# zhaorz/FlowOnTheGo

Measured on AMD Instinct MI355X. Metric: frame-pairs/sec @1080p DIS op-pt 2 (4 batches of 64 in flight), higher is better.
Workload: dtype f32; 1 GPU; BASELINE configs[2]: batch 64 synthetic 1920x1080 gray f32 pairs per GPU resident in HBM, DIS op-pt 2 + variational refinement (SOR order: lexicographic = the reference's order), output = finest-scale flow 120x68x2; global_batch=64, pairs_in_flight=256, batches_in_flight_per_gpu=4, parallelism=frame-pair sharding x1, no collective

## Files before the change

### flowonthego_amd/csrc/fotg_capi.hip

```cpp
#include <math.h>
#include <stdio.h>
#include <stdlib.h>
#include <string.h>
#include <atomic>
#include <map>
#include <mutex>
#include <new>
#include <type_traits>
#include "host_call.h"
#include "pipe_tickets.h"
#include "pipe_queues.h"
#include "pyramid.hip.h"
#include "lk.hip.h"
#include "lk_fast.hip.h"
#include "densify.hip.h"
#include "varref.hip.h"
#include "varref_tiles.hip.h"
#include "varref_levelpipe.hip.h"
#include "varref_depth.hip.h"
#include "upsample.hip.h"

using namespace fotg;

static thread_local int g_last_hip = 0;
// ... 1 lines not shown
#define HIPCHK(x)                                   \
  do {                                              \
    hipError_t e_ = (x);                            \
    if (e_ != hipSuccess) { g_last_hip = (int)e_; return FOTG_ERR_HIP; } \
  } while (0)
#define LAUNCHCHK() HIPCHK(hipGetLastError())

#define ON_DEVICE(dev)                                                              \
  DevGuard dev_guard_(dev);                                                         \
  if (!dev_guard_.ok) { g_last_hip = (int)hipGetLastError(); return FOTG_ERR_HIP; }

struct GridState {
  const float *I0, *I0x, *I0y, *I1;
  long stride;
  const float *flow_prev;
  float *trace_host;
  int camlr;
};
struct Grid {
  float *p_iter[FOTG_MAXLEV];
  float *pweight[FOTG_MAXLEV];
  GridState gs[FOTG_MAXLEV];
};
struct PyrBufs {
  float *im[FOTG_MAXLEV], *dx[FOTG_MAXLEV], *dy[FOTG_MAXLEV];
};

struct FotgTune {
  int vr_path;
  int vr_stream;
  int vr_levelpipe;
  int lp_max_pairs;
  int vr_first_data;
  int pyr_split;
  int lk_shw;
  int lk_lpp;
  int lk_banded;
  int lk_fast_r;
  int lk_lpp_min_waves;
  int test_taps;
};
static const char *env_str(const char *name) { return getenv(name); }
static int env_int(const char *name, int dflt) { const char *e = env_str(name); return e ? atoi(e) : dflt; }

#ifdef FOTG_DEBUG
static std::map<void *, void *> g_dbg_base;
static std::mutex g_dbg_mu;
static hipError_t fotg_dbg_free(void *p)
{
  void *base = p;
  { std::lock_guard<std::mutex> g(g_dbg_mu); auto it = g_dbg_base.find(p); if (it != g_dbg_base.end()) { base = it->second; g_dbg_base.erase(it); } }
  return (hipFree)(base);
}
#define hipFree(p) fotg_dbg_free((void *)(p))
#endif
struct fotg_ctx {
#ifdef FOTG_DEBUG
  struct Guard { const char *name; char *begin, *end; size_t size; } guards[256];
  int nguards;
#endif
  fotg_params p;
  FotgTune tune;
  int w_org, h_org, Wp, Hp, padw, padh, device, max_batch, noc, ps;
  int nch;
  int base_lv;
  LevelGeom geom[FOTG_MAXLEV];
  PyrBufs pyr[2];
  long lev_stride[FOTG_MAXLEV];
  float *flow[FOTG_MAXLEV];
  Grid fw;
  Grid bw;
  float *flow_bw[FOTG_MAXLEV];
  float *tap_t[FOTG_MAXLEV], *tap_tx[FOTG_MAXLEV], *tap_ty[FOTG_MAXLEV], *tap_hes[FOTG_MAXLEV];
  int *tap_cnt[FOTG_MAXLEV];
  float *trace_dev[FOTG_MAXLEV];
  bool taps;
  float *vr;
  long vr_pair_stride;
  float4 *vrC[FOTG_MAXLEV];
  float2 *vrD[FOTG_MAXLEV];
  VrArgs vra[FOTG_MAXLEV];
  int verbosity;
  hipEvent_t tev[4 * FOTG_MAXLEV + 4];
  float tt[FOTG_MAXLEV][5];
  float tt_pyr, tt_total;
  float2 *vrX[FOTG_MAXLEV];
  long x_pair_stride[FOTG_MAXLEV];
  int x_rt[FOTG_MAXLEV];
  int *tileSync;
  long sync_total;
  int tile_nbs;
  int lp_ntr;
  int *stall_host, *stall_dev;
  long stalls;
  unsigned long long *stamps;
};
// ... 94 lines not shown
    (void)hipFree(c->trace_dev[l]);
    (void)hipFree(c->vrC[l]); (void)hipFree(c->vrD[l]); (void)hipFree(c->vrX[l]);
  }
  if (c->stall_host) (void)hipHostFree(c->stall_host);
  (void)hipFree(c->vr); (void)hipFree(c->tileSync); (void)hipFree(c->stamps);
  for (auto &e : c->tev) if (e) (void)hipEventDestroy(e);
  delete c;
}

int fotg_create(const fotg_params *p, int w_org, int h_org, int device, int max_batch, fotg_ctx **out)
{
  if (!p || !out || w_org <= 0 || h_org <= 0 || max_batch <= 0) return FOTG_ERR_ARG;
  if (p->noc != 1 && p->noc != 3) return FOTG_ERR_ARG;
  if (p->ps != 4 && p->ps != 8 && p->ps != 12 && p->ps != 16) return FOTG_ERR_UNSUPPORTED;
  if (p->sc_l < 0 || p->sc_f < p->sc_l || p->sc_f >= FOTG_MAXLEV) return FOTG_ERR_ARG;
  if (p->max_iter < 0 || p->tv_solverit < 0 || p->tv_innerit < 0) return FOTG_ERR_ARG;
  if (p->costfct < 0 || p->costfct > 2 || (p->costfct == 2 && !(p->normoutlier > 0))) return FOTG_ERR_ARG;
  if (p->depth && p->usetvref && p->sor_mode != FOTG_SOR_LEXICOGRAPHIC) return FOTG_ERR_UNSUPPORTED;
  if (p->sor_mode < FOTG_SOR_LEXICOGRAPHIC || p->sor_mode > FOTG_SOR_POINT) return FOTG_ERR_ARG;
  if (p->u8_color < 0 || p->u8_color > 2 || (p->u8_color && p->noc != 1)) return FOTG_ERR_ARG;
  if (p->bidir != 0 && p->bidir != 1) return FOTG_ERR_ARG;
  if (p->bidir && p->depth) return FOTG_ERR_UNSUPPORTED;
  ON_DEVICE(device);
  fotg_ctx *c = new (std::nothrow) fotg_ctx();
  if (!c) return FOTG_ERR_ARG;
  memset((void *)c, 0, sizeof(*c));
  c->p = *p; c->w_org = w_org; c->h_org = h_org; c->device = device; c->max_batch = max_batch;
  c->noc = p->noc; c->ps = p->ps; c->nch = p->depth ? 1 : 2;
  c->tune.vr_path = env_int("FOTG_VR_PATH", 0);
  c->tune.vr_stream = env_int("FOTG_VR_STREAM", 1);
  c->tune.vr_levelpipe = env_int("FOTG_VR_LEVELPIPE", 1);
  c->tune.lp_max_pairs = env_int("FOTG_VR_LEVELPIPE_MAX_PAIRS", 1 << 20);
  c->tune.vr_first_data = env_int("FOTG_VR_FIRST_DATA", 1);
  c->tune.pyr_split = env_int("FOTG_PYR_SPLIT", 1);
  c->tune.test_taps = env_int("FOTG_TEST_TAPS", 0);
  c->tune.lk_shw = env_int("FOTG_LK_SHW", -1);
  c->tune.lk_lpp = env_int("FOTG_LK_LPP", 0);
  c->tune.lk_banded = env_int("FOTG_LK_BANDED", 1);
  c->tune.lk_lpp_min_waves = env_int("FOTG_LK_LPP_MIN_WAVES", 2048);
  c->tune.lk_fast_r = env_int("FOTG_LK_FAST_R", 2);
  if (hipHostMalloc((void **)&c->stall_host, 64, hipHostMallocMapped) != hipSuccess ||
      hipHostGetDevicePointer((void **)&c->stall_dev, c->stall_host, 0) != hipSuccess) { g_last_hip = (int)hipGetLastError(); fotg_destroy(c); return FOTG_ERR_HIP; }
  memset(c->stall_host, 0, 64);
  fotg_padded_size(w_org, h_org, p->sc_f, &c->Wp, &c->Hp, &c->padw, &c->padh);
  c->base_lv = p->sc_l < 4 ? p->sc_l : 4;
  const size_t B = (size_t)max_batch;
  for (int l = c->base_lv; l <= p->sc_f; ++l) {
    LevelGeom &g = c->geom[l];
    fill_geom(*p, c->Wp, c->Hp, l, g);
    if (g.w < 1 || g.h < 1) { fotg_destroy(c); return FOTG_ERR_ARG; }
    c->lev_stride[l] = (long)g.tw * g.th * c->noc;
    const size_t bytes = B * c->lev_stride[l] * sizeof(float);
#ifdef FOTG_DEBUG
#define FOTG_GUARD_BYTES 65536
#define ALLOC(ptr, nbytes) do { const bool gd_ = getenv("FOTG_DEBUG_GUARD") != nullptr; const size_t nb_ = ((nbytes) + 255) & ~(size_t)255; char *base_ = nullptr; \
    if (hipMalloc((void **)&base_, nb_ + (gd_ ? 2 * FOTG_GUARD_BYTES : 0)) != hipSuccess) { g_last_hip = (int)hipGetLastError(); fotg_destroy(c); return FOTG_ERR_HIP; } \
    *(void **)&(ptr) = gd_ ? base_ + FOTG_GUARD_BYTES : base_; \
    if (getenv("FOTG_DEBUG_POISON")) (void)hipMemset((ptr), getenv("FOTG_DEBUG_POISON")[0] == '2' ? 0x4B : 0xFF, nb_); \
    if (gd_ && c->nguards < 256) { (void)hipMemset(base_, 0xA5, FOTG_GUARD_BYTES); (void)hipMemset(base_ + FOTG_GUARD_BYTES + nb_, 0xA5, FOTG_GUARD_BYTES); \
      { std::lock_guard<std::mutex> g_(g_dbg_mu); g_dbg_base[(void *)(ptr)] = base_; } \
      c->guards[c->nguards].name = #ptr; c->guards[c->nguards].begin = base_; c->guards[c->nguards].end = base_ + FOTG_GUARD_BYTES + nb_; c->guards[c->nguards++].size = nb_; } } while (0)
#else
#define ALLOC(ptr, nbytes) do { if (hipMalloc((void **)&(ptr), (nbytes)) != hipSuccess) { g_last_hip = (int)hipGetLastError(); fotg_destroy(c); return FOTG_ERR_HIP; } } while (0)
#endif
    const size_t bytes1 = (B + 1) * c->lev_stride[l] * sizeof(float);
    ALLOC(c->pyr[0].im[l], bytes1);
// ... 533 lines not shown
  const int npx = a.w * a.h;
  if (mode != FOTG_SOR_POINT && c->tune.vr_path == 0 && inner >= 1 && sync_bands(a, sweeps) == 1 && fused_lds_bytes(a, false) <= 156 * 1024 &&
      (npx <= 3000 || mode == FOTG_SOR_REDBLACK)) {
    p.nsweeps = nosor ? 0 : sweeps;
    p.fused = fused_lds_bytes(a, true) > FOTG_LDS_MAX ? FUSED_CGLOBAL
            : c->noc == 1 && npx > 1024 && npx <= 2048 ? FUSED_RES1024
            : c->noc == 1 && npx <= 1024 ? FUSED_RES
            : FUSED_CL;
    p.lds = fused_lds_bytes(a, p.fused != FUSED_CGLOBAL);
    return p;
  }
  p.merged_first = c->tune.vr_first_data && inner > 0;
  const bool tiled = c->vrX[l] && c->tileSync;
  const int ntr = (a.h + FOTG_LP_TH - 1) / FOTG_LP_TH;
  const long lp_words = lp_tile_words(n, c->tile_nbs) + lp_data_words(n, ntr);
  p.levelpipe = tiled && c->tune.vr_levelpipe && n <= c->tune.lp_max_pairs && c->tune.vr_path == 0 && c->tune.vr_first_data &&
                inner >= 1 && inner <= FOTG_LP_KMAX && sweeps >= 2 && sweeps <= 4 && ntr <= c->lp_ntr && lp_words <= c->sync_total;
  p.zsync_n = !tiled ? 0 : p.levelpipe ? (int)lp_words : (int)tile_sync_words(n, c->tile_nbs);
  if (p.levelpipe) {
    const int nb = (a.h + FOTG_TILE_ROWS - 1) / FOTG_TILE_ROWS;
    p.lp_nwg = (unsigned)n * (unsigned)(inner * nb * sweeps + (inner - 1) * ntr * FOTG_LP_DW);
    p.excl = (p.lp_nwg <= 256 && !((c->tune.vr_levelpipe >> 4) & 8)) ? 72 * 1024 : 0;
  }
  return p;
}

template <typename... A>
static int opt_in_lds(void (*fn)(A...), int lds)
{
  HIPCHK(lds_opt_in(fn, lds));
  return FOTG_OK;
}

enum LaunchCount { CNT_SOR_STREAM, CNT_SOR_PIPE, CNT_FUSED_CGLOBAL, CNT_SOR_TILES, CNT_SOR_TALL, CNT_LEVEL_PIPE, CNT_N };
static const char *const g_count_name[CNT_N] = {"sor_stream", "sor_pipe", "fused_cglobal", "sor_tiles", "sor_tall", "level_pipe"};
static std::atomic<long> g_count[CNT_N];

#ifndef FOTG_TILE_P
#define FOTG_TILE_P 8
#endif
static TileArgs tile_args(const fotg_ctx *c, int l, int n)
{
  const VrArgs &a = c->vra[l];
  return {c->vrX[l], c->x_pair_stride[l], (long)(a.S + 1 + FOTG_TILE_DUMP) * c->x_rt[l], c->x_rt[l], (a.h + FOTG_TILE_ROWS - 1) / FOTG_TILE_ROWS, n,
          c->tileSync, c->tile_nbs, c->tileSync + c->sync_total, c->stall_dev};
}

template <int K, int P, bool POINT = false>
static void launch_sor_wave(const VrArgs &a, int n, int sweeps, float omega, hipStream_t s)
{
  constexpr int U = POINT ? (K <= 4 ? 4 : 1) : (K <= 2) ? (P >= 8 ? 64 : 8 * P) : (K <= 4 ? 4 * P : P);
  vr_sor_kernel<K, P, U, POINT><<<n, 64, 0, s>>>(a, sweeps, omega);
}

template <bool FM>
static int run_sor(fotg_ctx *c, int l, int n, const SorPlan &q, bool zeroed, hipStream_t s)
{
  const VrArgs &a = c->vra[l];
  const int sweeps = c->p.tv_solverit;
  const float omega = c->p.tv_sor;
  int st = FOTG_OK;
  switch (q.kind) {
    case SOR_NONE: return FOTG_OK;
    case SOR_STREAM70:
      if ((st = opt_in_lds(vr_sor_stream_kernel<72, 70, FOTG_SYNC_M, kVrU, FM>, q.lds))) return st;
      vr_sor_stream_kernel<72, 70, FOTG_SYNC_M, kVrU, FM><<<n, 1024, q.lds, s>>>(with_bands(a, q.nsweeps, q.nbands), omega);
      ++g_count[CNT_SOR_STREAM];
      break;
    case SOR_STREAM98:
// ... 64 lines not shown

template <int NOC, bool FM>
static int varref_impl(fotg_ctx *c, int l, int n, const float *I0, const float *I1, long img_stride, float *flow, hipStream_t s)
{
  const LevelGeom &g = c->geom[l];
  const VrArgs &a = c->vra[l];
  const long fs = (long)g.w * g.h * 2;
  dim3 grid((g.w * g.h + 255) / 256, n), block(256);
  const float quarter_alpha = 0.25f * c->p.tv_alpha;
  const float half_gamma_over3 = c->p.tv_gamma * 0.5f / 3.0f;
  const float half_delta_over3 = c->p.tv_delta * 0.5f / 3.0f;
  const int inner = c->p.tv_innerit * (l + 1);
  const VrPlan p = plan_level(c, l, n);
  int st = FOTG_OK;
  if (p.fused != FUSED_NONE) {
    VrArgs b = with_bands(a, p.nsweeps, 1);
    b.taps = c->taps ? 1 : 0;
    b.redblack = c->p.sor_mode == FOTG_SOR_REDBLACK;
    const auto fused = [&](auto launch) {
      return launch(b, p.lds, n, s, inner, quarter_alpha, half_delta_over3, half_gamma_over3, c->p.tv_sor, flow, fs, I0, I1, img_stride, g.tw, c->ps);
    };
    switch (p.fused) {
      case FUSED_RES1024: if constexpr (NOC == 1) st = fused(launch_fused<1, true, true, 1024, FM>); break;
      case FUSED_RES: if constexpr (NOC == 1) st = fused(launch_fused<1, true, true, 512, FM>); break;
      case FUSED_CL: st = fused(launch_fused<NOC, true, false, 512, FM>); break;
      default: st = fused(launch_fused<NOC, false, false, 512, FM>); ++g_count[CNT_FUSED_CGLOBAL]; break;
    }
    if (st) return st;
    LAUNCHCHK();
    return FOTG_OK;
  }
  VrArgs az = a;
  if (p.zsync_n) { az.zsync = c->tileSync; az.zsync_n = p.zsync_n; }
  {
    dim3 gs_(((g.w + 31) / 32) * ((g.h + 7) / 8), n);
    if ((n & 7) != 0 && gs_.x >= 256 && c->tune.lk_banded) { az.nwg = (int)gs_.x; gs_.x = (gs_.x + 7) & ~7u; }
    vr_setup_kernel<NOC, 2, FM><<<gs_, 256, 0, s>>>(az, I0, I1, img_stride, g.tw, c->ps, flow, fs, 1, p.merged_first ? 1 : 0, quarter_alpha, half_delta_over3, half_gamma_over3);
    LAUNCHCHK();
  }
  if (p.levelpipe) {
    LevelPipeArgs q;
    q.K = inner; q.ntr = (g.h + FOTG_LP_TH - 1) / FOTG_LP_TH; q.tiles_x = (g.w + FOTG_TW - 1) / FOTG_TW;
    q.dprog = c->tileSync + lp_tile_words(n, c->tile_nbs);
    q.quarter_alpha = quarter_alpha; q.half_delta_over3 = half_delta_over3; q.half_gamma_over3 = half_gamma_over3;
    q.dbg = c->tune.vr_levelpipe >> 4;
    q.stamps = nullptr;
    if (q.dbg & 4) {
      if (!c->stamps && hipMalloc((void **)&c->stamps, 8 * 8 * 8192) != hipSuccess) return FOTG_ERR_HIP;
      (void)hipMemsetAsync(c->stamps, 0, 8 * 8 * 8192, s);
      q.stamps = (long long *)c->stamps;
    }
    if (p.excl && (st = opt_in_lds(vr_level_pipe_kernel<NOC, FOTG_TILE_P, FM>, p.excl))) return st;
    vr_level_pipe_kernel<NOC, FOTG_TILE_P, FM><<<p.lp_nwg, 256, p.excl, s>>>(a, tile_args(c, l, n), q, c->p.tv_solverit, c->p.tv_sor);
    LAUNCHCHK();
    ++g_count[CNT_LEVEL_PIPE];
    vr_finish_kernel<<<grid, block, 0, s>>>(a, flow, fs);
    LAUNCHCHK();
    return FOTG_OK;
  }
  for (int it = 0; it < inner; ++it) {
    if (!(it == 0 && p.merged_first)) {
      vr_data_kernel<NOC, FM><<<dim3(((g.w + FOTG_TW - 1) / FOTG_TW) * ((g.h + FOTG_TH - 1) / FOTG_TH), n), 256, 0, s>>>(az, quarter_alpha, half_delta_over3, half_gamma_over3);
      LAUNCHCHK();
    }
    if ((st = run_sor<FM>(c, l, n, p.sor, p.zsync_n != 0, s))) return st;
  }
  vr_finish_kernel<<<grid, block, 0, s>>>(a, flow, fs);
  LAUNCHCHK();
  return FOTG_OK;
}

// ... 17 lines not shown
  else if (split && p.lds_mode) p.kind = DE_SPLIT;
  else p.kind = c->p.tv_solverit == 3 ? DE_SW3 : DE_SW1;
  return p;
}

template <int SW, bool SPLIT = false>
static int launch_de_sor(const VrArgs &a, int n, const DePlan &p, float omega, int camlr, hipStream_t s)
{
  const int nt = SPLIT ? 3 * p.threads : p.threads;
  int st = FOTG_OK;
  switch (p.lds_mode) {
    case 2: if (!(st = opt_in_lds(vr_de_sor_kernel<SW, 2, SPLIT>, p.lds))) vr_de_sor_kernel<SW, 2, SPLIT><<<n, nt, p.lds, s>>>(a, omega, camlr); break;
    case 1: if (!(st = opt_in_lds(vr_de_sor_kernel<SW, 1, SPLIT>, p.lds))) vr_de_sor_kernel<SW, 1, SPLIT><<<n, nt, p.lds, s>>>(a, omega, camlr); break;
    default: if constexpr (!SPLIT) vr_de_sor_kernel<SW, 0><<<n, nt, 0, s>>>(a, omega, camlr); break;
  }
  return st;
}

template <int NOC>
static int varref_depth_impl(fotg_ctx *c, int l, int n, const float *I0, const float *I1, long img_stride, float *flow, hipStream_t s, int camlr)
{
  const LevelGeom &g = c->geom[l];
  const VrArgs &a = c->vra[l];
  const long fs = (long)g.w * g.h;
  dim3 grid((g.w * g.h + 255) / 256, n), block(256);
  const float quarter_alpha = 0.25f * c->p.tv_alpha;
  const float half_gamma_over3 = c->p.tv_gamma * 0.5f / 3.0f;
  const float half_delta_over3 = c->p.tv_delta * 0.5f / 3.0f;
  const int inner = c->p.tv_innerit * (l + 1);
  const int sweeps = c->p.tv_solverit;
  const float omega = c->p.tv_sor;
  const DePlan p = plan_depth(c, l);
  int st = FOTG_OK;
  vr_setup_kernel<NOC, 1><<<dim3(((g.w + 31) / 32) * ((g.h + 7) / 8), n), 256, 0, s>>>(a, I0, I1, img_stride, g.tw, c->ps, flow, fs);
  LAUNCHCHK();
  if (p.kind == DE_INNER) {
    if ((st = opt_in_lds(vr_de_inner_kernel<NOC>, p.lds))) return st;
    vr_de_inner_kernel<NOC><<<n, 1024, p.lds, s>>>(a, inner, quarter_alpha, half_delta_over3, half_gamma_over3, omega, camlr, flow, fs, p.threads, c->taps ? 1 : 0);
    LAUNCHCHK();
    return FOTG_OK;
  }
  vr_de_init_kernel<<<grid, block, 0, s>>>(a);
  LAUNCHCHK();
  for (int it = 0; it < inner; ++it) {
    vr_de_smooth_kernel<<<grid, block, 0, s>>>(a, quarter_alpha);
    LAUNCHCHK();
    vr_de_data_kernel<NOC><<<grid, block, 0, s>>>(a, half_delta_over3, half_gamma_over3);
    LAUNCHCHK();
    switch (p.kind) {
      case DE_TALL:
        for (int k = 0; k < sweeps; ++k) vr_de_sor_tall_kernel<<<n, 1024, 0, s>>>(a, omega, camlr, k == sweeps - 1 ? 1 : 0);
        break;
      case DE_SPLIT: st = launch_de_sor<3, true>(a, n, p, omega, camlr, s); break;
      case DE_SW3: st = launch_de_sor<3>(a, n, p, omega, camlr, s); break;
      default: for (int k = 0; k < sweeps && !st; ++k) st = launch_de_sor<1>(a, n, p, omega, camlr, s); break;
    }
    if (st) return st;
    LAUNCHCHK();
  }
  vr_de_finish_kernel<<<grid, block, 0, s>>>(a, flow, fs);
  LAUNCHCHK();
  return FOTG_OK;
}

static int varref_dispatch(fotg_ctx *c, int l, int n, const float *I0, const float *I1, long pair_stride, float *flow, hipStream_t stream, int camlr)
{
  int st = check_level(c, l, n); if (st) return st;
  if (!I0 || !I1 || !flow || !c->vr) return FOTG_ERR_ARG;
// ... 703 lines not shown
```

### flowonthego_amd/csrc/varref.hip.h

```cpp
#pragma once
#include <type_traits>
#include "common.h"

namespace fotg {

enum VrPlane { P_WX = 0, P_WY, P_MASK, P_NSINGLE };
enum VrCPlane { C_AVG = 0, C_IZ, C_IX, C_IY, C_IXX, C_IXY, C_IYY, C_IXZ, C_IYZ, C_NCOLOR };

struct VrArgs {
  float *base;
  long pair_stride;
  long pl;
  int w, h, st, noc;
  float4 *C;
  float2 *D;
  long c_pair_stride;
  long d_pair_stride;
  int S, SC, RP, RPD, K, nlanes, nsweeps, nbands, band_rows, band_mode, taps;
  int *zsync;
  int zsync_n;
  int nwg;
  int redblack;
  int point;
  __host__ __device__ int pix(int i, int j) const { return j * st + i; }
// ... 72 lines not shown
__device__ __forceinline__ void prep_pixel(const VrArgs &a, int pair, int i, int j, const float *__restrict__ I0, const float *__restrict__ I1,
                                           long img_stride, int tw, int pad, const float *__restrict__ flow, long flow_stride)
{
  prep_store<NOC>(a, pair, i, j, prep_values<NOC>(a, pair, i, j, I0, I1, img_stride, tw, pad, flow, flow_stride));
}

template <int NOC>
__device__ __forceinline__ void deriv1_pixel(const VrArgs &a, int pair, int i, int j)
{
  const int o = j * a.st + i;
#pragma unroll
  for (int c = 0; c < NOC; ++c) {
    const float *avg = a.color(pair, C_AVG, c), *iz = a.color(pair, C_IZ, c);
    a.color(pair, C_IX, c)[o] = conv_h5(avg + (size_t)j * a.st, i, a.w);
    a.color(pair, C_IY, c)[o] = conv_v5(avg + i, j, a.h, a.st);
    a.color(pair, C_IXZ, c)[o] = conv_h5(iz + (size_t)j * a.st, i, a.w);
    a.color(pair, C_IYZ, c)[o] = conv_v5(iz + i, j, a.h, a.st);
  }
}

template <int NOC>
__device__ __forceinline__ void deriv2_pixel(const VrArgs &a, int pair, int i, int j)
{
  const int o = j * a.st + i;
#pragma unroll
  for (int c = 0; c < NOC; ++c) {
    const float *ix = a.color(pair, C_IX, c), *iy = a.color(pair, C_IY, c);
    a.color(pair, C_IXX, c)[o] = conv_h5(ix + (size_t)j * a.st, i, a.w);
    a.color(pair, C_IXY, c)[o] = conv_v5(ix + i, j, a.h, a.st);
    a.color(pair, C_IYY, c)[o] = conv_v5(iy + i, j, a.h, a.st);
  }
}

template <int NOC, int NCH, bool FM>
__device__ __forceinline__ void first_data_term(const VrArgs &a, int pair, int tx0, int ty0, const float *__restrict__ flow, long flow_stride,
                                                float quarter_alpha, float half_delta_over3, float half_gamma_over3);

template <int NOC, int NCH = 2, bool FM = false>
__global__ __launch_bounds__(256) void vr_setup_kernel(VrArgs a, const float *__restrict__ I0, const float *__restrict__ I1,
                                                       long img_stride, int tw, int pad,
                                                       const float *__restrict__ flow, long flow_stride, int zero_d = 0,
                                                       int first_data = 0, float quarter_alpha = 0.f, float half_delta_over3 = 0.f, float half_gamma_over3 = 0.f)
{
  constexpr int TW_ = 32, TH_ = 8, XW = TW_ + 8, XH = TH_ + 8, YW = TW_ + 4, YH = TH_ + 4;
  __shared__ float Xa[NOC][XH * XW], Xz[NOC][XH * XW], Yx[NOC][YH * YW], Yy[NOC][YH * YW];
  if (first_data && a.zsync_n > 0)
    for (long k = ((long)blockIdx.y * gridDim.x + blockIdx.x) * 256 + threadIdx.x; k < a.zsync_n; k += (long)gridDim.x * gridDim.y * 256) a.zsync[k] = 0;
  WgId wg = xcd_local_wg();
  int ntiles = (int)gridDim.x;
  if (a.nwg > 0) { wg.x = xcd_banded_x(a.nwg); ntiles = a.nwg; if (wg.x < 0) return; }
  const int pair = wg.y, w = a.w, h = a.h;
  const int tiles_x = (w + TW_ - 1) / TW_;
  if (zero_d == 1) {
    float2 *D = a.Dp(pair);
    for (long k = (long)wg.x * 256 + threadIdx.x; k < a.d_pair_stride; k += (long)ntiles * 256) D[k] = make_float2(0.f, 0.f);
  }
  const int tx0 = (wg.x % tiles_x) * TW_, ty0 = (wg.x / tiles_x) * TH_;
  for (int e = threadIdx.x; e < XW * XH; e += 256) {
    const int cx = tx0 - 4 + e % XW, cy = ty0 - 4 + e / XW;
    const int gx = clampi(cx, w), gy = clampi(cy, h);
    const PrepVal<NOC> v = prep_values<NOC, NCH>(a, pair, gx, gy, I0, I1, img_stride, tw, pad, flow, flow_stride);
#pragma unroll
    for (int c = 0; c < NOC; ++c) { Xa[c][e] = v.avg[c]; Xz[c][e] = v.iz[c]; }
    if (cx >= tx0 && cx < tx0 + TW_ && cy >= ty0 && cy < ty0 + TH_ && cx < w && cy < h) prep_store<NOC>(a, pair, cx, cy, v);
  }
  __syncthreads();
  for (int e = threadIdx.x; e < YW * YH; e += 256) {
    const int cx = tx0 - 2 + e % YW, cy = ty0 - 2 + e / YW;
    const int gx = clampi(cx, w), gy = clampi(cy, h);
    const bool own = cx >= tx0 && cx < tx0 + TW_ && cy >= ty0 && cy < ty0 + TH_ && cx < w && cy < h;
#pragma unroll
    for (int c = 0; c < NOC; ++c) {
      const float *arow = Xa[c] + (gy - ty0 + 4) * XW - tx0 + 4, *acol = Xa[c] + (4 - ty0) * XW + gx - tx0 + 4;
      const float *zrow = Xz[c] + (gy - ty0 + 4) * XW - tx0 + 4, *zcol = Xz[c] + (4 - ty0) * XW + gx - tx0 + 4;
      const float ix = conv_h5(arow, gx, w), iy = conv_v5(acol, gy, h, XW);
      const float ixz = conv_h5(zrow, gx, w), iyz = conv_v5(zcol, gy, h, XW);
      Yx[c][e] = ix; Yy[c][e] = iy;
      if (own) {
        const int o = a.pix(cx, cy);
        a.color(pair, C_IX, c)[o] = ix; a.color(pair, C_IY, c)[o] = iy; a.color(pair, C_IXZ, c)[o] = ixz; a.color(pair, C_IYZ, c)[o] = iyz;
      }
    }
  }
  __syncthreads();
  const int i = tx0 + (threadIdx.x % TW_), j = ty0 + (threadIdx.x / TW_);
  if (i < w && j < h) {
    const int o = a.pix(i, j);
#pragma unroll
    for (int c = 0; c < NOC; ++c) {
      const float *xrow = Yx[c] + (j - ty0 + 2) * YW - tx0 + 2, *xcol = Yx[c] + (2 - ty0) * YW + i - tx0 + 2, *ycol = Yy[c] + (2 - ty0) * YW + i - tx0 + 2;
      a.color(pair, C_IXX, c)[o] = conv_h5(xrow, i, w);
      a.color(pair, C_IXY, c)[o] = conv_v5(xcol, j, h, YW);
      a.color(pair, C_IYY, c)[o] = conv_v5(ycol, j, h, YW);
    }
  }
  if constexpr (NCH == 2) {
    if (first_data) {
      __syncthreads();
      first_data_term<NOC, NCH, FM>(a, pair, tx0, ty0, flow, flow_stride, quarter_alpha, half_delta_over3, half_gamma_over3);
    }
  }
}

template <int NOC>
struct PixIn {
  float Ix[NOC], Iy[NOC], Iz[NOC], Ixx[NOC], Ixy[NOC], Iyy[NOC], Ixz[NOC], Iyz[NOC];
  float m, wxc, wxl, wxr, wxt, wxb, wyc, wyl, wyr, wyt, wyb;
  __device__ __forceinline__ float dxl() const { return wxc - wxl; }
  __device__ __forceinline__ float dxr() const { return wxr - wxc; }
  __device__ __forceinline__ float dxt() const { return wxc - wxt; }
  __device__ __forceinline__ float dxb() const { return wxb - wxc; }
  __device__ __forceinline__ float dyl() const { return wyc - wyl; }
  __device__ __forceinline__ float dyr() const { return wyr - wyc; }
  __device__ __forceinline__ float dyt() const { return wyc - wyt; }
  __device__ __forceinline__ float dyb() const { return wyb - wyc; }
};
template <int NOC>
__device__ __forceinline__ PixIn<NOC> data_load(const VrArgs &a, int pair, int i, int j)
{
  const int st = a.st, w = a.w, h = a.h, o = j * st + i;
  const float *wx = a.single(pair, P_WX), *wy = a.single(pair, P_WY);
  PixIn<NOC> p;
#pragma unroll
  for (int c = 0; c < NOC; ++c) {
    p.Ix[c] = a.color(pair, C_IX, c)[o]; p.Iy[c] = a.color(pair, C_IY, c)[o]; p.Iz[c] = a.color(pair, C_IZ, c)[o];
    p.Ixx[c] = a.color(pair, C_IXX, c)[o]; p.Ixy[c] = a.color(pair, C_IXY, c)[o]; p.Iyy[c] = a.color(pair, C_IYY, c)[o];
    p.Ixz[c] = a.color(pair, C_IXZ, c)[o]; p.Iyz[c] = a.color(pair, C_IYZ, c)[o];
  }
  p.m = a.single(pair, P_MASK)[o];
  const int ol = i > 0 ? o - 1 : o, orr = i < w - 1 ? o + 1 : o, ot = j > 0 ? o - st : o, ob = j < h - 1 ? o + st : o;
  p.wxc = wx[o]; p.wxl = wx[ol]; p.wxr = wx[orr]; p.wxt = wx[ot]; p.wxb = wx[ob];
  p.wyc = wy[o]; p.wyl = wy[ol]; p.wyr = wy[orr]; p.wyt = wy[ot]; p.wyb = wy[ob];
  return p;
// ... 51 lines not shown
  const int x0 = (tile % tiles_x) * FOTG_TW, y0 = (tile / tiles_x) * FOTG_TH;
  const int lx = threadIdx.x % FOTG_TW, ly = threadIdx.x / FOTG_TW;
  const int i = x0 + lx, j = y0 + ly, o = j * st + i;
  const float *wx = a.single(pair, P_WX), *wy = a.single(pair, P_WY);
  const float2 *D = a.Dp(pair);
  const bool inimg = i < w && j < h;
  const int ic0 = inimg ? i : 0, jc0 = inimg ? j : 0;
  const PixIn<NOC> pin = data_load<NOC>(a, pair, ic0, jc0);
  const float2 duv = D[a.didx(ic0, jc0)];
  for (int k = threadIdx.x; k < UW * UH; k += 256) {
    const int jj = clampi(y0 - 2 + k / UW, h), ii = clampi(x0 - 2 + k % UW, w);
    const int q = jj * st + ii;
    const float2 d = D[a.didx(ii, jj)];
    uv[k] = make_float2(wx[q] + d.x, wy[q] + d.y);
  }
  __syncthreads();
  for (int k = threadIdx.x; k < SW * SH; k += 256) {
    const int sy = k / SW, sx = k % SW;
    const int c = (sy + 1) * UW + (sx + 1);
    sm[k] = smooth_w<FM>(uv[c - 1], uv[c], uv[c + 1], uv[c - UW], uv[c + UW], y0 - 1 + sy, h, quarter_alpha);
  }
  __syncthreads();
  if (i >= w || j >= h) return;
  const int sc = (ly + 1) * SW + (lx + 1);
  const float s_o = sm[sc];
  const float hr = (i < w - 1) ? s_o + sm[sc + 1] : 0.0f;
  const float hl = (i > 0) ? sm[sc - 1] + s_o : 0.0f;
  const float vb = (j < h - 1) ? s_o + sm[sc + SW] : 0.0f;
  const float vt = (j > 0) ? sm[sc - SW] + s_o : 0.0f;

  data_term_compute<NOC, FM>(a, pair, i, j, pin, hr, hl, vb, vt, duv.x, duv.y, half_delta_over3, half_gamma_over3);
}

template <int NOC, int NCH, bool FM>
__device__ __forceinline__ void first_data_term(const VrArgs &a, int pair, int x0, int y0, const float *__restrict__ flow, long flow_stride,
                                                float quarter_alpha, float half_delta_over3, float half_gamma_over3)
{
  constexpr int UW = FOTG_TW + 4, UH = FOTG_TH + 4, SW = FOTG_TW + 2, SH = FOTG_TH + 2;
  __shared__ float2 uv[UW * UH];
  __shared__ float sm[SW * SH];
  const int st = a.st, w = a.w, h = a.h;
  const int lx = threadIdx.x % FOTG_TW, ly = threadIdx.x / FOTG_TW;
  const int i = x0 + lx, j = y0 + ly;
  const float *fl = flow + (size_t)pair * flow_stride;
  auto W = [&](int ii, int jj) { const float *f = fl + NCH * (size_t)(jj * w + ii); return make_float2(f[0], f[NCH - 1]); };
  for (int k = threadIdx.x; k < UW * UH; k += 256) {
    const float2 wv = W(clampi(x0 - 2 + k % UW, w), clampi(y0 - 2 + k / UW, h));
    uv[k] = make_float2(wv.x + 0.f, wv.y + 0.f);
  }
  __syncthreads();
  for (int k = threadIdx.x; k < SW * SH; k += 256) {
    const int sy = k / SW, sx = k % SW;
    const int c = (sy + 1) * UW + (sx + 1);
    sm[k] = smooth_w<FM>(uv[c - 1], uv[c], uv[c + 1], uv[c - UW], uv[c + UW], y0 - 1 + sy, h, quarter_alpha);
  }
  __syncthreads();
  if (i >= w || j >= h) return;
  const int sc = (ly + 1) * SW + (lx + 1), o = j * st + i;
  const float s_o = sm[sc];
  const float hr = (i < w - 1) ? s_o + sm[sc + 1] : 0.0f;
  const float hl = (i > 0) ? sm[sc - 1] + s_o : 0.0f;
  const float vb = (j < h - 1) ? s_o + sm[sc + SW] : 0.0f;
  const float vt = (j > 0) ? sm[sc - SW] + s_o : 0.0f;
  PixIn<NOC> p;
#pragma unroll
  for (int c = 0; c < NOC; ++c) {
    p.Ix[c] = a.color(pair, C_IX, c)[o]; p.Iy[c] = a.color(pair, C_IY, c)[o]; p.Iz[c] = a.color(pair, C_IZ, c)[o];
    p.Ixx[c] = a.color(pair, C_IXX, c)[o]; p.Ixy[c] = a.color(pair, C_IXY, c)[o]; p.Iyy[c] = a.color(pair, C_IYY, c)[o];
    p.Ixz[c] = a.color(pair, C_IXZ, c)[o]; p.Iyz[c] = a.color(pair, C_IYZ, c)[o];
  }
  p.m = a.single(pair, P_MASK)[o];
  const float2 wc = W(i, j), wl = W(i > 0 ? i - 1 : i, j), wr = W(i < w - 1 ? i + 1 : i, j), wt = W(i, j > 0 ? j - 1 : j), wb = W(i, j < h - 1 ? j + 1 : j);
  p.wxc = wc.x; p.wxl = wl.x; p.wxr = wr.x; p.wxt = wt.x; p.wxb = wb.x;
  p.wyc = wc.y; p.wyl = wl.y; p.wyr = wr.y; p.wyt = wt.y; p.wyb = wb.y;
  data_term_compute<NOC, FM>(a, pair, i, j, p, hr, hl, vb, vt, 0.f, 0.f, half_delta_over3, half_gamma_over3);
}

__device__ __forceinline__ float2 sor_update(float2 cur, float4 c0, float4 c1, float hl, float2 left, float2 top, float2 right, float2 bottom, float omega)
{
  const float a11 = c0.x, a12 = c0.y, b1 = c0.z, b2 = c0.w, a22 = c1.x, hr = c1.y, vb = c1.z, vt = c1.w;
  float s1 = hr * right.x, s2 = hr * right.y;
  s1 = s1 + vt * top.x;    s2 = s2 + vt * top.y;
  s1 = s1 + vb * bottom.x; s2 = s2 + vb * bottom.y;
  s1 = s1 + b1;            s2 = s2 + b2;
  const float B1 = hl * left.x + s1, B2 = hl * left.y + s2;
  float2 r;
  r.x = cur.x + omega * (a11 * B1 + a12 * B2 - cur.x);
  r.y = cur.y + omega * (a12 * B1 + a22 * B2 - cur.y);
  return r;
}

__device__ __forceinline__ float2 sor_update_point(float2 cur, float4 c0, float4 c1, float hl, float2 left, float2 top, float2 right, float2 bottom, float omega)
{
  const float A11 = c0.x, A12 = c0.y, b1 = c0.z, b2 = c0.w, A22 = c1.x, hr = c1.y, vb = c1.z, vt = c1.w;
  float su = 0.0f - vt * top.x, sv = 0.0f - vt * top.y;
  su = su - hl * left.x;   sv = sv - hl * left.y;
  su = su - vb * bottom.x; sv = sv - vb * bottom.y;
  su = su - hr * right.x;  sv = sv - hr * right.y;
  const float B1 = b1 - su, B2 = b2 - sv;
  float2 r;
  r.x = (1.0f - omega) * cur.x + omega / A11 * (B1 - A12 * cur.y);
  r.y = (1.0f - omega) * cur.y + omega / A22 * (B2 - A12 * r.x);
  const bool live = omega != 0.f && A11 != 0.f;
  r.x = live ? r.x : cur.x;
// ... 716 lines not shown
```

Measured before the change: 181,800 frame-pairs/s.

## Template varref setup tile shape and pass first-data inputs through registers

Templates the variational-refinement setup kernel on tile width and height, adds a 30x17 tile alongside 32x8, and picks between them at runtime. The choice weighs halo overhead against occupancy rounds across the device's compute units. The fused first-data term now takes its per-pixel derivative and mask inputs from shared memory and registers filled during setup, instead of re-reading them from global memory. The gain is less halo recompute and fewer global loads, at the cost of extra shared memory per workgroup, which can lower occupancy.

```diff
diff --git a/flowonthego_amd/csrc/fotg_capi.hip b/flowonthego_amd/csrc/fotg_capi.hip
--- a/flowonthego_amd/csrc/fotg_capi.hip
+++ b/flowonthego_amd/csrc/fotg_capi.hip
@@ -57,6 +57,7 @@
   int vr_levelpipe;
   int lp_max_pairs;
   int vr_first_data;
+  int vr_tile;
   int pyr_split;
   int lk_shw;
   int lk_lpp;
@@ -87,6 +88,7 @@
   fotg_params p;
   FotgTune tune;
   int w_org, h_org, Wp, Hp, padw, padh, device, max_batch, noc, ps;
+  int ncu;
   int nch;
   int base_lv;
   LevelGeom geom[FOTG_MAXLEV];
@@ -247,6 +249,8 @@
   c->tune.vr_levelpipe = env_int("FOTG_VR_LEVELPIPE", 1);
   c->tune.lp_max_pairs = env_int("FOTG_VR_LEVELPIPE_MAX_PAIRS", 1 << 20);
   c->tune.vr_first_data = env_int("FOTG_VR_FIRST_DATA", 1);
+  c->tune.vr_tile = env_int("FOTG_VR_TILE", 0);
+  if (hipDeviceGetAttribute(&c->ncu, hipDeviceAttributeMultiprocessorCount, device) != hipSuccess || c->ncu < 1) c->ncu = 1;
   c->tune.pyr_split = env_int("FOTG_PYR_SPLIT", 1);
   c->tune.test_taps = env_int("FOTG_TEST_TAPS", 0);
   c->tune.lk_shw = env_int("FOTG_LK_SHW", -1);
@@ -846,9 +850,43 @@
   return FOTG_OK;
 }
 
-enum LaunchCount { CNT_SOR_STREAM, CNT_SOR_PIPE, CNT_FUSED_CGLOBAL, CNT_SOR_TILES, CNT_SOR_TALL, CNT_LEVEL_PIPE, CNT_N };
-static const char *const g_count_name[CNT_N] = {"sor_stream", "sor_pipe", "fused_cglobal", "sor_tiles", "sor_tall", "level_pipe"};
+enum LaunchCount { CNT_SOR_STREAM, CNT_SOR_PIPE, CNT_FUSED_CGLOBAL, CNT_SOR_TILES, CNT_SOR_TALL, CNT_LEVEL_PIPE, CNT_SETUP, CNT_SETUP_LAST = CNT_SETUP + 1, CNT_N };
+static const char *const g_count_name[CNT_N] = {"sor_stream", "sor_pipe", "fused_cglobal", "sor_tiles", "sor_tall", "level_pipe", "setup_32x8", "setup_30x17"};
 static std::atomic<long> g_count[CNT_N];
+
+enum VrTile { VT_32x8, VT_30x17, VT_N };
+static_assert(CNT_SETUP_LAST == CNT_SETUP + VT_N - 1, "one set-up launch counter per tile shape");
+#define FOTG_VR_TILES(X) switch (tile) { case VT_30x17: X(30, 17); break; default: X(32, 8); break; }
+static const int kVrTileW[VT_N] = {32, 30}, kVrTileH[VT_N] = {8, 17};
+static long vr_tile_count(int w, int h, int t) { return (long)((w + kVrTileW[t] - 1) / kVrTileW[t]) * ((h + kVrTileH[t] - 1) / kVrTileH[t]); }
+static long vr_tile_cost(int w, int h, int t)
+{
+  const long tiles = vr_tile_count(w, h, t);
+  return tiles * (kVrTileW[t] + 8) * (kVrTileH[t] + 8) + tiles * vr_tile_threads(kVrTileW[t], kVrTileH[t]) - (long)w * h;
+}
+template <int NOC, int NCH, bool FM>
+static int vr_tile_shape(const fotg_ctx *c, int l, int n)
+{
+  if (c->tune.vr_tile > 0) return c->tune.vr_tile <= VT_N ? c->tune.vr_tile - 1 : VT_32x8;
+  struct Occ { int wgs[VT_N]; };
+  static const Occ occ = [] {
+    Occ o;
+    for (int tile = 0; tile < VT_N; ++tile) {
+      const void *fn = nullptr;
+#define FN(TW_, TH_) fn = (const void *)vr_setup_kernel<NOC, NCH, FM, TW_, TH_>
+      FOTG_VR_TILES(FN)
+#undef FN
+      if (hipOccupancyMaxActiveBlocksPerMultiprocessor(&o.wgs[tile], fn, vr_tile_threads(kVrTileW[tile], kVrTileH[tile]), 0) != hipSuccess) o.wgs[tile] = 0;
+    }
+    return o;
+  }();
+  const VrArgs &a = c->vra[l];
+  const auto rounds = [&](int t) { const long res = (long)occ.wgs[t] * c->ncu; return res > 0 ? (n * vr_tile_count(a.w, a.h, t) + res - 1) / res : -1; };
+  int best = VT_32x8;
+  for (int t = 1; t < VT_N; ++t)
+    if (vr_tile_cost(a.w, a.h, t) < vr_tile_cost(a.w, a.h, best) && rounds(t) > 0 && (rounds(VT_32x8) < 0 || rounds(t) <= rounds(VT_32x8))) best = t;
+  return best;
+}
 
 #ifndef FOTG_TILE_P
 #define FOTG_TILE_P 8
@@ -979,11 +1017,15 @@
   }
   VrArgs az = a;
   if (p.zsync_n) { az.zsync = c->tileSync; az.zsync_n = p.zsync_n; }
+  const int tile = vr_tile_shape<NOC, 2, FM>(c, l, n);
   {
-    dim3 gs_(((g.w + 31) / 32) * ((g.h + 7) / 8), n);
+    dim3 gs_((unsigned)vr_tile_count(g.w, g.h, tile), n);
     if ((n & 7) != 0 && gs_.x >= 256 && c->tune.lk_banded) { az.nwg = (int)gs_.x; gs_.x = (gs_.x + 7) & ~7u; }
-    vr_setup_kernel<NOC, 2, FM><<<gs_, 256, 0, s>>>(az, I0, I1, img_stride, g.tw, c->ps, flow, fs, 1, p.merged_first ? 1 : 0, quarter_alpha, half_delta_over3, half_gamma_over3);
+#define SETUP(TW_, TH_) vr_setup_kernel<NOC, 2, FM, TW_, TH_><<<gs_, vr_tile_threads(TW_, TH_), 0, s>>>(az, I0, I1, img_stride, g.tw, c->ps, flow, fs, 1, p.merged_first ? 1 : 0, quarter_alpha, half_delta_over3, half_gamma_over3)
+    FOTG_VR_TILES(SETUP)
+#undef SETUP
     LAUNCHCHK();
+    ++g_count[CNT_SETUP + tile];
   }
   if (p.levelpipe) {
     LevelPipeArgs q;
@@ -1067,8 +1109,12 @@
   const float omega = c->p.tv_sor;
   const DePlan p = plan_depth(c, l);
   int st = FOTG_OK;
-  vr_setup_kernel<NOC, 1><<<dim3(((g.w + 31) / 32) * ((g.h + 7) / 8), n), 256, 0, s>>>(a, I0, I1, img_stride, g.tw, c->ps, flow, fs);
+  const int tile = vr_tile_shape<NOC, 1, false>(c, l, n);
+#define SETUP(TW_, TH_) vr_setup_kernel<NOC, 1, false, TW_, TH_><<<dim3((unsigned)vr_tile_count(g.w, g.h, tile), n), vr_tile_threads(TW_, TH_), 0, s>>>(a, I0, I1, img_stride, g.tw, c->ps, flow, fs)
+  FOTG_VR_TILES(SETUP)
+#undef SETUP
   LAUNCHCHK();
+  ++g_count[CNT_SETUP + tile];
   if (p.kind == DE_INNER) {
     if ((st = opt_in_lds(vr_de_inner_kernel<NOC>, p.lds))) return st;
     vr_de_inner_kernel<NOC><<<n, 1024, p.lds, s>>>(a, inner, quarter_alpha, half_delta_over3, half_gamma_over3, omega, camlr, flow, fs, p.threads, c->taps ? 1 : 0);
diff --git a/flowonthego_amd/csrc/varref.hip.h b/flowonthego_amd/csrc/varref.hip.h
--- a/flowonthego_amd/csrc/varref.hip.h
+++ b/flowonthego_amd/csrc/varref.hip.h
@@ -128,20 +128,26 @@
   }
 }
 
-template <int NOC, int NCH, bool FM>
+template <int NOC>
+struct PixIn;
+template <int NOC, int NCH, bool FM, int TW_, int TH_>
 __device__ __forceinline__ void first_data_term(const VrArgs &a, int pair, int tx0, int ty0, const float *__restrict__ flow, long flow_stride,
-                                                float quarter_alpha, float half_delta_over3, float half_gamma_over3);
-
-template <int NOC, int NCH = 2, bool FM = false>
-__global__ __launch_bounds__(256) void vr_setup_kernel(VrArgs a, const float *__restrict__ I0, const float *__restrict__ I1,
+                                                float quarter_alpha, float half_delta_over3, float half_gamma_over3, PixIn<NOC> &p);
+
+__host__ __device__ constexpr int vr_tile_threads(int tw, int th) { return (tw * th + 63) / 64 * 64; }
+
+template <int NOC, int NCH = 2, bool FM = false, int TW_ = 32, int TH_ = 8>
+__global__ __launch_bounds__(vr_tile_threads(TW_, TH_)) void vr_setup_kernel(VrArgs a, const float *__restrict__ I0, const float *__restrict__ I1,
                                                        long img_stride, int tw, int pad,
                                                        const float *__restrict__ flow, long flow_stride, int zero_d = 0,
                                                        int first_data = 0, float quarter_alpha = 0.f, float half_delta_over3 = 0.f, float half_gamma_over3 = 0.f)
 {
-  constexpr int TW_ = 32, TH_ = 8, XW = TW_ + 8, XH = TH_ + 8, YW = TW_ + 4, YH = TH_ + 4;
+  constexpr int NT = vr_tile_threads(TW_, TH_), XW = TW_ + 8, XH = TH_ + 8, YW = TW_ + 4, YH = TH_ + 4;
+  constexpr bool FD = NCH == 2;
   __shared__ float Xa[NOC][XH * XW], Xz[NOC][XH * XW], Yx[NOC][YH * YW], Yy[NOC][YH * YW];
+  __shared__ float Zm[FD ? TW_ * TH_ : 1], Zx[NOC][FD ? TW_ * TH_ : 1], Zy[NOC][FD ? TW_ * TH_ : 1];
   if (first_data && a.zsync_n > 0)
-    for (long k = ((long)blockIdx.y * gridDim.x + blockIdx.x) * 256 + threadIdx.x; k < a.zsync_n; k += (long)gridDim.x * gridDim.y * 256) a.zsync[k] = 0;
+    for (long k = ((long)blockIdx.y * gridDim.x + blockIdx.x) * NT + threadIdx.x; k < a.zsync_n; k += (long)gridDim.x * gridDim.y * NT) a.zsync[k] = 0;
   WgId wg = xcd_local_wg();
   int ntiles = (int)gridDim.x;
   if (a.nwg > 0) { wg.x = xcd_banded_x(a.nwg); ntiles = a.nwg; if (wg.x < 0) return; }
@@ -149,19 +155,22 @@
   const int tiles_x = (w + TW_ - 1) / TW_;
   if (zero_d == 1) {
     float2 *D = a.Dp(pair);
-    for (long k = (long)wg.x * 256 + threadIdx.x; k < a.d_pair_stride; k += (long)ntiles * 256) D[k] = make_float2(0.f, 0.f);
+    for (long k = (long)wg.x * NT + threadIdx.x; k < a.d_pair_stride; k += (long)ntiles * NT) D[k] = make_float2(0.f, 0.f);
   }
   const int tx0 = (wg.x % tiles_x) * TW_, ty0 = (wg.x / tiles_x) * TH_;
-  for (int e = threadIdx.x; e < XW * XH; e += 256) {
+  for (int e = threadIdx.x; e < XW * XH; e += NT) {
     const int cx = tx0 - 4 + e % XW, cy = ty0 - 4 + e / XW;
     const int gx = clampi(cx, w), gy = clampi(cy, h);
     const PrepVal<NOC> v = prep_values<NOC, NCH>(a, pair, gx, gy, I0, I1, img_stride, tw, pad, flow, flow_stride);
 #pragma unroll
     for (int c = 0; c < NOC; ++c) { Xa[c][e] = v.avg[c]; Xz[c][e] = v.iz[c]; }
-    if (cx >= tx0 && cx < tx0 + TW_ && cy >= ty0 && cy < ty0 + TH_ && cx < w && cy < h) prep_store<NOC>(a, pair, cx, cy, v);
+    if (cx >= tx0 && cx < tx0 + TW_ && cy >= ty0 && cy < ty0 + TH_ && cx < w && cy < h) {
+      prep_store<NOC>(a, pair, cx, cy, v);
+      if constexpr (FD) Zm[(cy - ty0) * TW_ + cx - tx0] = v.mask;
+    }
   }
   __syncthreads();
-  for (int e = threadIdx.x; e < YW * YH; e += 256) {
+  for (int e = threadIdx.x; e < YW * YH; e += NT) {
     const int cx = tx0 - 2 + e % YW, cy = ty0 - 2 + e / YW;
     const int gx = clampi(cx, w), gy = clampi(cy, h);
     const bool own = cx >= tx0 && cx < tx0 + TW_ && cy >= ty0 && cy < ty0 + TH_ && cx < w && cy < h;
@@ -175,26 +184,33 @@
       if (own) {
         const int o = a.pix(cx, cy);
         a.color(pair, C_IX, c)[o] = ix; a.color(pair, C_IY, c)[o] = iy; a.color(pair, C_IXZ, c)[o] = ixz; a.color(pair, C_IYZ, c)[o] = iyz;
+        if constexpr (FD) { Zx[c][(cy - ty0) * TW_ + cx - tx0] = ixz; Zy[c][(cy - ty0) * TW_ + cx - tx0] = iyz; }
       }
     }
   }
   __syncthreads();
-  const int i = tx0 + (threadIdx.x % TW_), j = ty0 + (threadIdx.x / TW_);
-  if (i < w && j < h) {
+  const int lx = threadIdx.x % TW_, ly = threadIdx.x / TW_;
+  const int i = tx0 + lx, j = ty0 + ly;
+  PixIn<NOC> pin;
+  if (ly < TH_ && i < w && j < h) {
     const int o = a.pix(i, j);
 #pragma unroll
     for (int c = 0; c < NOC; ++c) {
       const float *xrow = Yx[c] + (j - ty0 + 2) * YW - tx0 + 2, *xcol = Yx[c] + (2 - ty0) * YW + i - tx0 + 2, *ycol = Yy[c] + (2 - ty0) * YW + i - tx0 + 2;
-      a.color(pair, C_IXX, c)[o] = conv_h5(xrow, i, w);
-      a.color(pair, C_IXY, c)[o] = conv_v5(xcol, j, h, YW);
-      a.color(pair, C_IYY, c)[o] = conv_v5(ycol, j, h, YW);
-    }
-  }
-  if constexpr (NCH == 2) {
-    if (first_data) {
-      __syncthreads();
-      first_data_term<NOC, NCH, FM>(a, pair, tx0, ty0, flow, flow_stride, quarter_alpha, half_delta_over3, half_gamma_over3);
-    }
+      const float ixx = conv_h5(xrow, i, w), ixy = conv_v5(xcol, j, h, YW), iyy = conv_v5(ycol, j, h, YW);
+      a.color(pair, C_IXX, c)[o] = ixx;
+      a.color(pair, C_IXY, c)[o] = ixy;
+      a.color(pair, C_IYY, c)[o] = iyy;
+      if constexpr (FD) {
+        pin.Ixx[c] = ixx; pin.Ixy[c] = ixy; pin.Iyy[c] = iyy;
+        pin.Ix[c] = Yx[c][(ly + 2) * YW + lx + 2]; pin.Iy[c] = Yy[c][(ly + 2) * YW + lx + 2]; pin.Iz[c] = Xz[c][(ly + 4) * XW + lx + 4];
+        pin.Ixz[c] = Zx[c][ly * TW_ + lx]; pin.Iyz[c] = Zy[c][ly * TW_ + lx];
+      }
+    }
+    if constexpr (FD) pin.m = Zm[ly * TW_ + lx];
+  }
+  if constexpr (FD) {
+    if (first_data) first_data_term<NOC, NCH, FM, TW_, TH_>(a, pair, tx0, ty0, flow, flow_stride, quarter_alpha, half_delta_over3, half_gamma_over3, pin);
   }
 }
 
@@ -312,44 +328,36 @@
   data_term_compute<NOC, FM>(a, pair, i, j, pin, hr, hl, vb, vt, duv.x, duv.y, half_delta_over3, half_gamma_over3);
 }
 
-template <int NOC, int NCH, bool FM>
+template <int NOC, int NCH, bool FM, int TW_, int TH_>
 __device__ __forceinline__ void first_data_term(const VrArgs &a, int pair, int x0, int y0, const float *__restrict__ flow, long flow_stride,
-                                                float quarter_alpha, float half_delta_over3, float half_gamma_over3)
-{
-  constexpr int UW = FOTG_TW + 4, UH = FOTG_TH + 4, SW = FOTG_TW + 2, SH = FOTG_TH + 2;
+                                                float quarter_alpha, float half_delta_over3, float half_gamma_over3, PixIn<NOC> &p)
+{
+  constexpr int NT = vr_tile_threads(TW_, TH_), UW = TW_ + 4, UH = TH_ + 4, SW = TW_ + 2, SH = TH_ + 2;
   __shared__ float2 uv[UW * UH];
   __shared__ float sm[SW * SH];
-  const int st = a.st, w = a.w, h = a.h;
-  const int lx = threadIdx.x % FOTG_TW, ly = threadIdx.x / FOTG_TW;
+  const int w = a.w, h = a.h;
+  const int lx = threadIdx.x % TW_, ly = threadIdx.x / TW_;
   const int i = x0 + lx, j = y0 + ly;
   const float *fl = flow + (size_t)pair * flow_stride;
   auto W = [&](int ii, int jj) { const float *f = fl + NCH * (size_t)(jj * w + ii); return make_float2(f[0], f[NCH - 1]); };
-  for (int k = threadIdx.x; k < UW * UH; k += 256) {
+  for (int k = threadIdx.x; k < UW * UH; k += NT) {
     const float2 wv = W(clampi(x0 - 2 + k % UW, w), clampi(y0 - 2 + k / UW, h));
     uv[k] = make_float2(wv.x + 0.f, wv.y + 0.f);
   }
   __syncthreads();
-  for (int k = threadIdx.x; k < SW * SH; k += 256) {
+  for (int k = threadIdx.x; k < SW * SH; k += NT) {
     const int sy = k / SW, sx = k % SW;
     const int c = (sy + 1) * UW + (sx + 1);
     sm[k] = smooth_w<FM>(uv[c - 1], uv[c], uv[c + 1], uv[c - UW], uv[c + UW], y0 - 1 + sy, h, quarter_alpha);
   }
   __syncthreads();
-  if (i >= w || j >= h) return;
-  const int sc = (ly + 1) * SW + (lx + 1), o = j * st + i;
+  if (ly >= TH_ || i >= w || j >= h) return;
+  const int sc = (ly + 1) * SW + (lx + 1);
   const float s_o = sm[sc];
   const float hr = (i < w - 1) ? s_o + sm[sc + 1] : 0.0f;
   const float hl = (i > 0) ? sm[sc - 1] + s_o : 0.0f;
   const float vb = (j < h - 1) ? s_o + sm[sc + SW] : 0.0f;
   const float vt = (j > 0) ? sm[sc - SW] + s_o : 0.0f;
-  PixIn<NOC> p;
-#pragma unroll
-  for (int c = 0; c < NOC; ++c) {
-    p.Ix[c] = a.color(pair, C_IX, c)[o]; p.Iy[c] = a.color(pair, C_IY, c)[o]; p.Iz[c] = a.color(pair, C_IZ, c)[o];
-    p.Ixx[c] = a.color(pair, C_IXX, c)[o]; p.Ixy[c] = a.color(pair, C_IXY, c)[o]; p.Iyy[c] = a.color(pair, C_IYY, c)[o];
-    p.Ixz[c] = a.color(pair, C_IXZ, c)[o]; p.Iyz[c] = a.color(pair, C_IYZ, c)[o];
-  }
-  p.m = a.single(pair, P_MASK)[o];
   const float2 wc = W(i, j), wl = W(i > 0 ? i - 1 : i, j), wr = W(i < w - 1 ? i + 1 : i, j), wt = W(i, j > 0 ? j - 1 : j), wb = W(i, j < h - 1 ? j + 1 : j);
   p.wxc = wc.x; p.wxl = wl.x; p.wxr = wr.x; p.wxt = wt.x; p.wxb = wb.x;
   p.wyc = wc.y; p.wyl = wl.y; p.wyr = wr.y; p.wyt = wt.y; p.wyb = wb.y;
```

Result: faster. 187,000 frame-pairs/s (median of 4 runs) (+2.9%).
